# moxime/joint-vae

Hardware: AMD Instinct MI355X
Metric: training_images_per_sec (higher is better)
Workload: dtype f32

## Files before the change

### include/jvae_hip.h

```cpp
#ifndef JVAE_HIP_H
#define JVAE_HIP_H

#include <stddef.h>

#ifdef __cplusplus
extern "C" {
#endif

const char* jvae_version(void);

int jvae_gemm_f32(int M, int N, int K, int batch,
                  const float* A, long sAm, long sAk, long sAb,
                  const float* B, long sBk, long sBn, long sBb,
                  float* C, long sCm, long sCn, long sCb,
                  const float* bias, int bias_mode, int flags, int splitk, void* stream);

int jvae_splitk_fold_f32(const float* part, const float* bias, float* y, int S, long MN, int N, int relu, int accumulate,
                         void* stream);

size_t jvae_conv2d_workspace_bytes(int N, int Cin, int H, int W, int Cout, int KH, int KW, int S, int P, int OP,
                                   int transposed);
int jvae_conv2d_set_split_bf16(int mode);
int jvae_conv2d_set_split_shape16(int on);
int jvae_conv2d_out_shape(int H, int W, int KH, int KW, int S, int P, int OP, int transposed, int* OH, int* OW);
int jvae_conv2d_fwd_f32(const float* x, const float* w, const float* bias, float* y,
                        int N, int Cin, int H, int W, int Cout, int KH, int KW, int S, int P, int OP, int transposed,
                        void* ws, size_t ws_bytes, void* stream);
int jvae_conv2d_stats_splits(int N, int Cin, int H, int W, int Cout, int KH, int KW, int S, int P, int OP, int transposed);
int jvae_conv2d_fwd_stats_f32(const float* x, const float* w, const float* bias, float* y, float* stats, int* nsplit,
                              int N, int Cin, int H, int W, int Cout, int KH, int KW, int S, int P, int OP, int transposed,
                              void* ws, size_t ws_bytes, void* stream);
int jvae_conv2d_dgrad_f32(const float* dy, const float* w, float* dx,
                          int N, int Cin, int H, int W, int Cout, int KH, int KW, int S, int P, int OP, int transposed,
                          void* ws, size_t ws_bytes, void* stream);
int jvae_conv2d_wgrad_f32(const float* x, const float* dy, float* dw, float* dbias, int accumulate,
                          int N, int Cin, int H, int W, int Cout, int KH, int KW, int S, int P, int OP, int transposed,
                          void* ws, size_t ws_bytes, void* stream);

int jvae_pack_cache_configure(void* buf, size_t bytes);
int jvae_pack_cache_begin(void* stream, long long owner, const void* const* weights, int n);
int jvae_pack_cache_end(void);
int jvae_pack_cache_pin(void);
int jvae_pack_cache_reset(void);
int jvae_pack_cache_stats(int* entries, long long* hits, long long* misses, long long* refreshes);

size_t jvae_channel_sum_workspace_bytes(int C);
int jvae_channel_sum_f32(const float* t, float* out, int N, int C, int P, int accumulate, void* ws, size_t ws_bytes,
                         void* stream);

size_t jvae_bn_workspace_bytes(int C);
int jvae_bn_plan(int N, int C, int P, int* nsplit, int* nchunk);
int jvae_image_range(int N, int parts, int j, int* nb, int* ne);
int jvae_bn_fwd_f32(const float* x, const float* gamma, const float* beta,
                    float* running_mean, float* running_var, long long* num_batches_tracked,
                    float* y, float* save_mean, float* save_invstd,
                    int N, int C, int P, float momentum, float eps, int training, int relu,
                    void* ws, size_t ws_bytes, void* stream);
int jvae_bn_fwd_ext_f32(const float* x, const float* gamma, const float* beta,
                        float* running_mean, float* running_var, long long* num_batches_tracked,
                        float* y, float* save_mean, float* save_invstd,
                        int N, int C, int P, float momentum, float eps, int training, int relu,
                        const float* ext_stats, int ext_nsplit, const float* ext_pivot,
                        void* ws, size_t ws_bytes, void* stream);
// ... 181 lines not shown
```

### joint-vae_amd/csrc/conv_api.hip

```cpp
#include "common.h"
#include "jvae_internal.h"
#include "conv_dispatch.h"

namespace {

inline ConvRoute route(const ConvGeom& g, int transposed, ConvDir dir, CallFlags f = {}) {
    return jvae_conv_route(g, transposed, dir, CONV_F32, f);
}

bool affine_ok(const ConvGeom& g, int transposed, ConvDir other, const ConvRoute& r) {
    return r.aff_ok && route(g, transposed, other, {false, false, false, 1}).aff_ok;
}

int fwd_f32(const float* x, const float* w, const float* bias, float* y, float* stats, int* nsplit, const InAff* aff,
            int N, int Cin, int H, int W, int Cout, int KH, int KW, int S, int P, int OP, int transposed,
            void* ws, size_t ws_bytes, void* stream) {
    ConvGeom g; int oh, ow;
    if (nsplit) *nsplit = 0;
    if (!jvae_make_geom(N, Cin, H, W, Cout, KH, KW, S, P, OP, transposed, &g, &oh, &ow)) return JVAE_EINVAL;
    const ConvRoute r = route(g, transposed, CONV_FWD, {bias != nullptr, stats != nullptr, false, jvae_aff_kind(aff)});
    if (aff && !affine_ok(g, transposed, CONV_WGRAD, r)) return JVAE_ENOTSUP;
    if (N == 0) return 0;
    if (jvae_ws_short(r, ws, ws_bytes)) return JVAE_EWORKSPACE;
    return jvae_conv_run_fwd(r, g, x, w, bias, y, (float*)ws, ws_bytes, (hipStream_t)stream, stats, nsplit, aff);
// ... 106 lines not shown

int jvae_conv2d_wgrad_f32(const float* x, const float* dy, float* dw, float* dbias, int accumulate,
                          int N, int Cin, int H, int W, int Cout, int KH, int KW, int S, int P, int OP, int transposed,
                          void* ws, size_t ws_bytes, void* stream) {
    return wgrad_f32(x, dy, dw, dbias, accumulate, nullptr, N, Cin, H, W, Cout, KH, KW, S, P, OP, transposed, ws, ws_bytes, stream);
}

size_t jvae_channel_sum_workspace_bytes(int C) { return jvae_channel_sum_ws_bytes(C); }

int jvae_channel_sum_f32(const float* t, float* out, int N, int C, int P, int accumulate, void* ws, size_t ws_bytes,
                         void* stream) {
    if (!t || !out || N < 0 || C <= 0 || P <= 0) return JVAE_EINVAL;
    return jvae_channel_sum(t, out, N, C, P, accumulate, (float*)ws, ws_bytes, (hipStream_t)stream);
}

}
```

### joint-vae_amd/csrc/conv_dispatch.h

```cpp
#pragma once
#include "common.h"
#include "jvae_internal.h"

size_t jvae_conv_generic_ws(const ConvGeom& g);
int jvae_fold_fwd(const ConvGeom& g, const float* xb, const float* w, const float* bias, float* ys,
                  float* ws, size_t ws_bytes, hipStream_t st);
int jvae_fold_bwd(const ConvGeom& g, const float* ys, const float* w, const float* bias, float* xb,
                  float* ws, size_t ws_bytes, hipStream_t st);
int jvae_fold_wgrad(const ConvGeom& g, const float* xb, const float* ys, float* dw,
                    float* ws, size_t ws_bytes, hipStream_t st);
size_t jvae_channel_sum_ws_bytes(int C);
int jvae_channel_sum(const float* t, float* out, int N, int C, int P, int accumulate, float* ws, size_t ws_bytes,
                     hipStream_t st);

bool jvae_conv5_fwd_ok(int Cin, int H, int W, int Cout, int OH, int OW, int S, int P);
size_t jvae_conv5_pack_floats(int Cin, int Cout);
int jvae_conv5_fwd(const float* in, const float* w, int swap, int flip, const float* bias, float* out,
                   int N, int Cin, int H, int W, int Cout, int OW, int S, int P, float* ws, hipStream_t st,
                   float* stats = nullptr, int* nsplit = nullptr, const InAff* aff = nullptr);
int jvae_conv5_fwd_max_splits(int N, int OW);

int jvae_conv5_pack(const float* w, float* wp, int C, int O, int swap, int flip, hipStream_t st);

bool jvae_conv5_x3_ok(int Cin, int H, int W, int Cout, int OH, int OW, int S, int P);
size_t jvae_conv5_x3_pack_bytes(int Cin, int Cout);
int jvae_conv5_x3_set(int mode);
int jvae_conv5_x3_set_shape16(int on);
bool jvae_conv5_x3_enabled();
// ... 76 lines not shown
```

### joint-vae_amd/csrc/conv_generic.hip

```cpp
#include "common.h"
#include "jvae_internal.h"

namespace {

__global__ __launch_bounds__(256) void unfold_kernel(const float* __restrict__ xb, float* __restrict__ col,
                                                     ConvGeom g, int n0, int nimg, long sn, long sk, long sq,
                                                     int kfast) {
    const int Kd = g.Cb * g.KH * g.KW, Ps = g.Hs * g.Ws;
    const long total = (long)nimg * Kd * Ps;
    for (long i = (long)blockIdx.x * blockDim.x + threadIdx.x; i < total; i += (long)gridDim.x * blockDim.x) {
        int n, k, q;
        if (kfast) { k = (int)(i % Kd); long r = i / Kd; n = (int)(r % nimg); q = (int)(r / nimg); }
        else       { q = (int)(i % Ps); long r = i / Ps; k = (int)(r % Kd);  n = (int)(r / Kd); }
        const int kw = k % g.KW, kh = (k / g.KW) % g.KH, cb = k / (g.KW * g.KH);
        const int hs = q / g.Ws, ws = q % g.Ws;
        const int hb = hs * g.S + kh - g.P, wb = ws * g.S + kw - g.P;
        float v = 0.f;
        if (hb >= 0 && hb < g.Hb && wb >= 0 && wb < g.Wb)
            v = xb[(((long)(n0 + n) * g.Cb + cb) * g.Hb + hb) * g.Wb + wb];
        col[(long)n * sn + (long)k * sk + (long)q * sq] = v;
    }
}

template <bool KFAST>
// ... 56 lines not shown
            if (hs >= g.Hs) continue;
            for (int kw = 0; kw < g.KW; ++kw) {
                const int tw = wb + g.P - kw;
                if (tw < 0 || tw % g.S) continue;
                const int ws = tw / g.S;
                if (ws >= g.Ws) continue;
                const int k = (cb * g.KH + kh) * g.KW + kw;
                acc += col[(long)n * sn + (long)k * sk + (long)(hs * g.Ws + ws) * sq];
            }
        }
        xb[(((long)(n0 + n) * g.Cb + cb) * g.Hb + hb) * g.Wb + wb] = acc;
    }
}

__global__ __launch_bounds__(256) void channel_sum_kernel(const float* __restrict__ t, float* __restrict__ partial,
                                                          int N, int C, int P, int nsplit) {
    __shared__ float red[17];
    const int c = blockIdx.x, sp = blockIdx.y;
    const ImageRange ir = image_range(N, nsplit, sp);
    const int nb = ir.nb, ne = ir.ne;
    float s = 0.f;
    if ((P & 3) == 0) {
        const int P4 = P >> 2;
        const long cnt = (long)(ne - nb) * P4;
        for (long i = threadIdx.x; i < cnt; i += blockDim.x) {
            const long n = nb + i / P4, q = i % P4;
            const f32x4 v = *reinterpret_cast<const f32x4*>(t + (n * C + c) * (long)P + q * 4);
            s += (v[0] + v[1]) + (v[2] + v[3]);
        }
    } else {
        const long cnt = (long)(ne - nb) * P;
        for (long i = threadIdx.x; i < cnt; i += blockDim.x) {
            const long n = nb + i / P, q = i % P;
            s += t[(n * C + c) * (long)P + q];
        }
    }
    s = block_sum(s, red);
    if (threadIdx.x == 0) partial[(long)c * nsplit + sp] = s;
}

__global__ void channel_fold_kernel(const float* __restrict__ partial, float* __restrict__ out, int C, int nsplit,
                                    int accumulate) {
    const int c = blockIdx.x * blockDim.x + threadIdx.x;
    if (c >= C) return;
    float s = 0.f;
    for (int k = 0; k < nsplit; ++k) s += partial[(long)c * nsplit + k];
    out[c] = (accumulate ? out[c] : 0.f) + s;
}

inline int fold_slab_images(const ConvGeom& g) {
    const long per = (long)g.Cb * g.Hb * g.Wb;
    long n = ((1L << 31) - 1) / (per > 0 ? per : 1);
    if (const char* e = getenv("JVAE_FOLD_SLAB")) { const long v = atol(e); if (v > 0 && v < n) n = v; }
// ... 187 lines not shown
    }
    const int chunk = chunk_images(g, ws_bytes);
    if (chunk < 1) return JVAE_EWORKSPACE;
    for (int n0 = 0; n0 < g.N; n0 += chunk) {
        const int ni = (g.N - n0 < chunk) ? g.N - n0 : chunk;
        { const int rc = launch_unfold(xb, ws, g, n0, ni, false, st); if (rc) return rc; }
        int rc = jvae_gemm_launch(g.Cs, Kd, Ps, ni, ys + (long)n0 * g.Cs * Ps, Ps, 1, (long)g.Cs * Ps,
                                  ws, 1, Ps, (long)Kd * Ps, dw, Kd, 1, 0, nullptr, 0, 4, 1, st);
        if (rc) return rc;
    }
    return 0;
}

size_t jvae_channel_sum_ws_bytes(int C) { return sizeof(float) * (size_t)(C > 0 ? C : 1) * 64; }

int jvae_channel_sum(const float* t, float* out, int N, int C, int P, int accumulate, float* ws, size_t ws_bytes,
                     hipStream_t st) {
    if (C <= 0) return 0;
    if (N <= 0) {
        if (!accumulate) {
            hipError_t e = hipMemsetAsync(out, 0, sizeof(float) * (size_t)C, st);
            if (e != hipSuccess) return (int)e;
        }
        return 0;
    }
    if (!ws || ws_bytes < jvae_channel_sum_ws_bytes(C)) return JVAE_EWORKSPACE;
    long work = (long)N * P;
    int ns = (int)(work / 4096);
    const int cap = (1024 + C - 1) / C;
    if (ns > cap) ns = cap;
    if (ns > 64) ns = 64;
    if (ns > N) ns = N;
    if (ns < 1) ns = 1;
    hipLaunchKernelGGL(channel_sum_kernel, dim3(C, ns), dim3(256), 0, st, t, ws, N, C, P, ns);
    JVAE_LAUNCH_CHECK();
    hipLaunchKernelGGL(channel_fold_kernel, dim3(cdiv(C, 64)), dim3(64), 0, st, (const float*)ws, out, C, ns, accumulate);
    JVAE_LAUNCH_CHECK();
    return 0;
}
```

### joint-vae_amd/csrc/gemm.hip

```cpp
#include <stdlib.h>
#include "common.h"
#include "conv_x3.h"
#include "jvae_internal.h"
#include "conv_dispatch.h"

namespace {

constexpr int BK = 32;
constexpr int KQ = BK / 4;

struct GemmP {
    const float* A; long sAm, sAk, sAb;
    const float* B; long sBk, sBn, sBb;
    float* C; long sCm, sCn, sCb;
    const float* bias;
    int bias_mode;
    int bias_div;
    int M, N, K;
    int splitk;
    int kchunk;
    int flags;
    long sCsplit;
    int vecA, vecB;
    int xcd;
};

template <bool VEC>
__device__ __forceinline__ f32x4 load4(const float* p, long stride, int i0, int lim, bool row_ok) {
    f32x4 v = {0.f, 0.f, 0.f, 0.f};
    if (!row_ok) return v;
    if (VEC) {
        if (i0 + 3 < lim) return *reinterpret_cast<const f32x4*>(p);
    }
#pragma unroll
    for (int j = 0; j < 4; ++j)
        if (i0 + j < lim) v[j] = p[j * stride];
    return v;
}

template <int BM, int BN, bool AK, bool BNC>
__global__ __launch_bounds__(256) void gemm_kernel(GemmP p) {
    constexpr int LDA = BM + 4, LDB = BN + 4;
    constexpr int WM = BM / 2, WN = BN / 2;
    constexpr int TM = WM / 32, TN = WN / 32;
    constexpr int GA = BM * BK / 4 / 256;
    constexpr int GB = BN * BK / 4 / 256;
    __shared__ float As[BK * LDA];
    __shared__ float Bs[BK * LDB];

    const int tid = threadIdx.x, lane = tid & 63, wave = tid >> 6;
    const int wm0 = (wave >> 1) * WM, wn0 = (wave & 1) * WN;
    const int m0 = blockIdx.y * BM, n0 = blockIdx.x * BN;
    const int batch = blockIdx.z / p.splitk, split = blockIdx.z % p.splitk;
    const int kbeg = split * p.kchunk;
    const int kend = min(p.K, kbeg + p.kchunk);
    const float* A = p.A + (long)batch * p.sAb;
    const float* B = p.B + (long)batch * p.sBb;
    float* C = p.C + (long)batch * p.sCb + ((p.flags & 8) ? (long)split * p.sCsplit : 0L);

    f32x16 acc[TM][TN];
#pragma unroll
    for (int i = 0; i < TM; ++i)
#pragma unroll
        for (int j = 0; j < TN; ++j)
#pragma unroll
            for (int r = 0; r < 16; ++r) acc[i][j][r] = 0.f;

    f32x4 ra[GA], rb[GB];

    auto gload = [&](int k0) {
#pragma unroll
        for (int g = 0; g < GA; ++g) {
            if (AK) {
// ... 69 lines not shown
#pragma unroll
            for (int i = 0; i < TM; ++i)
#pragma unroll
                for (int j = 0; j < TN; ++j)
                    acc[i][j] = __builtin_amdgcn_mfma_f32_32x32x2f32(a[i], b[j], acc[i][j], 0, 0, 0);
        }
    }

    const bool lead = (split == 0) && !(p.flags & 8);
#pragma unroll
    for (int i = 0; i < TM; ++i)
#pragma unroll
        for (int j = 0; j < TN; ++j) {
            const int n = n0 + wn0 + j * 32 + l31;
            if (n >= p.N) continue;
            float bn = (p.bias_mode == 1 && lead) ? p.bias[n / p.bias_div] : 0.f;
#pragma unroll
            for (int r = 0; r < 16; ++r) {
                const int m = m0 + wm0 + i * 32 + (r & 3) + 8 * (r >> 2) + 4 * half;
                if (m >= p.M) continue;
                float v = acc[i][j][r] + bn;
                if (p.bias_mode == 2 && lead) v += p.bias[m];
                float* dst = C + (long)m * p.sCm + (long)n * p.sCn;
                if (p.flags & 8) {
                    *dst = v;
                } else if (p.flags & 4) {
                    atomicAdd(dst, v);
                } else {
                    if (p.flags & 1) v += *dst;
                    if (p.flags & 2) v = fmaxf(v, 0.f);
                    *dst = v;
                }
            }
        }
}

template <int BM, int BN>
int launch_tile(const GemmP& p, int batch, hipStream_t st) {
    dim3 grid(cdiv(p.N, BN), cdiv(p.M, BM), batch * p.splitk), block(256);
    const bool ak = (p.sAk == 1), bnc = (p.sBn == 1);
    if (ak && bnc)       hipLaunchKernelGGL((gemm_kernel<BM, BN, true, true>), grid, block, 0, st, p);
    else if (ak && !bnc) hipLaunchKernelGGL((gemm_kernel<BM, BN, true, false>), grid, block, 0, st, p);
    else if (!ak && bnc) hipLaunchKernelGGL((gemm_kernel<BM, BN, false, true>), grid, block, 0, st, p);
    else                 hipLaunchKernelGGL((gemm_kernel<BM, BN, false, false>), grid, block, 0, st, p);
    JVAE_LAUNCH_CHECK();
    return 0;
}

inline bool aligned16(const void* p) { return (reinterpret_cast<uintptr_t>(p) & 15) == 0; }

typedef __bf16 gx_bf16x8 __attribute__((ext_vector_type(8)));
typedef __bf16 gx_bf16x4 __attribute__((ext_vector_type(4)));
typedef unsigned int gx_u32x2 __attribute__((ext_vector_type(2)));
typedef unsigned int gx_u32x4 __attribute__((ext_vector_type(4)));
// ... 24 lines not shown
    constexpr int KQX = BKX / 4;
    extern __shared__ __attribute__((aligned(16))) unsigned char gx_lds[];
    unsigned char* As = gx_lds;
    unsigned char* Bs = gx_lds + 3 * IA::BYTES;

    const int tid = threadIdx.x, lane = tid & 63, wave = tid >> 6;
    const int half = lane >> 5, l31 = lane & 31;
    const int cg = (lane >> 4) & 1, q4 = (lane & 15) >> 2, pp = lane & 3;
    const int wm0 = (wave >> 1) * 32, wn0 = (wave & 1) * 32;
    unsigned bx = blockIdx.x, by = blockIdx.y, bz = blockIdx.z;
    if (p.xcd) {
        const unsigned lin = (unsigned)xcd_tile(bx + gridDim.x * (by + gridDim.y * bz), gridDim.x * gridDim.y * gridDim.z);
        bx = lin % gridDim.x; by = (lin / gridDim.x) % gridDim.y; bz = lin / (gridDim.x * gridDim.y);
    }
    const int m0 = by * BM, n0 = bx * BN;
    const int batch = bz / p.splitk, split = bz % p.splitk;
    const int kbeg = split * p.kchunk;
    const int kend = min(p.K, kbeg + p.kchunk);
    const float* A = p.A + (long)batch * p.sAb;
    const float* B = p.B + (long)batch * p.sBb;
    float* C = p.C + (long)batch * p.sCb + ((p.flags & 8) ? (long)split * p.sCsplit : 0L);

    f32x16 acc;
#pragma unroll
    for (int r = 0; r < 16; ++r) acc[r] = 0.f;
    f32x4 ra[DEPTH][G4], rb[DEPTH][G4];

    auto coordA = [&](int g, int k0, int* fast, int* slow) {
        if (AK) { *fast = k0 + (tid % KQX) * 4; *slow = m0 + tid / KQX + g * (256 / KQX); }
        else    { *fast = m0 + (tid % 16) * 4;  *slow = k0 + tid / 16 + g * 16; }
    };
    auto coordB = [&](int g, int k0, int* fast, int* slow) {
        if (BNC) { *fast = n0 + (tid % 16) * 4;  *slow = k0 + tid / 16 + g * 16; }
        else     { *fast = k0 + (tid % KQX) * 4; *slow = n0 + tid / KQX + g * (256 / KQX); }
    };
    auto okA = [&](int fast, int slow) { return AK ? (fast < kend && slow < p.M) : (fast + 3 < p.M && slow < kend); };
// ... 110 lines not shown
        }
    } else {
        if (kbeg < kend) gload(0, kbeg);
        for (int k0 = kbeg; k0 < kend; k0 += BKX) {
            __syncthreads();
            lstore(0, k0);
            __syncthreads();
            if (k0 + BKX < kend) gload(0, k0 + BKX);
            multiply();
        }
    }

    const bool lead = (split == 0) && !(p.flags & 8);
    const int n = n0 + wn0 + l31;
    if (n >= p.N) return;
    const float bn = (p.bias_mode == 1 && lead) ? p.bias[n / p.bias_div] : 0.f;
#pragma unroll
    for (int r = 0; r < 16; ++r) {
        const int m = m0 + wm0 + (r & 3) + 8 * (r >> 2) + 4 * half;
        if (m >= p.M) continue;
        float v = acc[r] + bn;
        if (p.bias_mode == 2 && lead) v += p.bias[m];
        float* dst = C + (long)m * p.sCm + (long)n * p.sCn;
        if (p.flags & 8) {
            *dst = v;
        } else if (p.flags & 4) {
            atomicAdd(dst, v);
        } else {
            if (p.flags & 1) v += *dst;
            if (p.flags & 2) v = fmaxf(v, 0.f);
            *dst = v;
        }
    }
}

template <bool AK, bool BNC, int DEPTH>
int launch_x3_variant(const GemmP& p, int batch, hipStream_t st) {
    constexpr int LDS = 3 * (GxImg<AK>::BYTES + GxImg<!BNC>::BYTES);
    static bool attr_set = false;
    if (!attr_set) {
        hipError_t e = hipFuncSetAttribute(reinterpret_cast<const void*>(&gemm_x3_kernel<AK, BNC, DEPTH>),
                                           hipFuncAttributeMaxDynamicSharedMemorySize, LDS);
        if (e != hipSuccess) return (int)e;
        attr_set = true;
    }
    dim3 grid(cdiv(p.N, 64), cdiv(p.M, 64), batch * p.splitk), block(256);
    hipLaunchKernelGGL((gemm_x3_kernel<AK, BNC, DEPTH>), grid, block, LDS, st, p);
    JVAE_LAUNCH_CHECK();
    return 0;
}

template <bool AK, bool BNC>
int launch_x3_ab(const GemmP& p, int batch, hipStream_t st) {
    const bool deep = p.vecA && p.vecB && p.K % 4 == 0
                      && (AK || p.M % 4 == 0) && (!BNC || p.N % 4 == 0);
    if (deep) return launch_x3_variant<AK, BNC, 3>(p, batch, st);
    return launch_x3_variant<AK, BNC, 1>(p, batch, st);
}

int launch_x3(const GemmP& p0, int batch, hipStream_t st) {
    GemmP p = p0;
// ... 8 lines not shown
inline bool gemm_x3_on(int K) {
    return K >= 64 && jvae_conv5_x3_enabled();
}

}

int jvae_gemm_launch(int M, int N, int K, int batch,
                     const float* A, long sAm, long sAk, long sAb,
                     const float* B, long sBk, long sBn, long sBb,
                     float* C, long sCm, long sCn, long sCb,
                     const float* bias, int bias_mode, int flags, int splitk, hipStream_t st) {
    return jvae_gemm_launch_ex(M, N, K, batch, A, sAm, sAk, sAb, B, sBk, sBn, sBb, C, sCm, sCn, sCb, bias, bias_mode, 1,
                               flags, splitk, st);
}

int jvae_gemm_launch_ex(int M, int N, int K, int batch,
                        const float* A, long sAm, long sAk, long sAb,
                        const float* B, long sBk, long sBn, long sBb,
                        float* C, long sCm, long sCn, long sCb,
                        const float* bias, int bias_mode, int bias_div, int flags, int splitk, hipStream_t st) {
    if (M <= 0 || N <= 0 || batch <= 0) return 0;
    if (K < 0 || !A || !B || !C) return JVAE_EINVAL;
    if (bias_mode && !bias) return JVAE_EINVAL;
    GemmP p;
    p.A = A; p.sAm = sAm; p.sAk = sAk; p.sAb = sAb;
    p.B = B; p.sBk = sBk; p.sBn = sBn; p.sBb = sBb;
    p.C = C; p.sCm = sCm; p.sCn = sCn; p.sCb = sCb;
    p.bias = bias; p.bias_mode = bias_mode; p.bias_div = bias_div > 0 ? bias_div : 1;
    p.M = M; p.N = N; p.K = K;
    if (splitk < 1) splitk = 1;
    int ktiles = cdiv(K, BK);
    if (splitk > ktiles) splitk = ktiles > 0 ? ktiles : 1;
    p.kchunk = cdiv(ktiles, splitk) * BK;
    splitk = K > 0 ? cdiv(K, p.kchunk) : 1;
    p.splitk = splitk;
    p.flags = flags & ~8;
    p.sCsplit = 0;
    if (splitk > 1) {
        if (flags & 2) return JVAE_EINVAL;
        p.flags |= 4;
    }
    const bool ak = (sAk == 1), bnc = (sBn == 1);
    p.vecA = aligned16(A) && (sAb % 4 == 0) && (ak ? (sAm % 4 == 0) : (sAm == 1 && sAk % 4 == 0));
    p.vecB = aligned16(B) && (sBb % 4 == 0) && (bnc ? (sBk % 4 == 0) : (sBk == 1 && sBn % 4 == 0));
    if (gemm_x3_on(K)) return launch_x3(p, batch, st);
    const long tiles128 = (long)cdiv(M, 128) * cdiv(N, 128) * batch * splitk;
    if (M > 64 && N > 64 && tiles128 >= 512) return launch_tile<128, 128>(p, batch, st);
    return launch_tile<64, 64>(p, batch, st);
}

int jvae_gemm_launch_part(int M, int N, int K, int batch,
                          const float* A, long sAm, long sAk, long sAb,
                          const float* B, long sBk, long sBn, long sBb,
                          float* part, long sCm, long sCn, long sCb, long sCsplit, int want_splits, int* splits,
                          hipStream_t st) {
    if (splits) *splits = 0;
    if (M <= 0 || N <= 0 || batch <= 0) return 0;
    if (K <= 0 || !A || !B || !part || !splits) return JVAE_EINVAL;
    GemmP p;
    p.A = A; p.sAm = sAm; p.sAk = sAk; p.sAb = sAb;
    p.B = B; p.sBk = sBk; p.sBn = sBn; p.sBb = sBb;
    p.C = part; p.sCm = sCm; p.sCn = sCn; p.sCb = sCb;
    p.bias = nullptr; p.bias_mode = 0; p.bias_div = 1;
    p.M = M; p.N = N; p.K = K;
    int splitk = want_splits < 1 ? 1 : want_splits;
    const int ktiles = cdiv(K, BK);
    if (splitk > ktiles) splitk = ktiles;
    p.kchunk = cdiv(ktiles, splitk) * BK;
    splitk = cdiv(K, p.kchunk);
    p.splitk = splitk;
    p.flags = 8;
    p.sCsplit = sCsplit;
    const bool ak = (sAk == 1), bnc = (sBn == 1);
    p.vecA = aligned16(A) && (sAb % 4 == 0) && (ak ? (sAm % 4 == 0) : (sAm == 1 && sAk % 4 == 0));
    p.vecB = aligned16(B) && (sBb % 4 == 0) && (bnc ? (sBk % 4 == 0) : (sBk == 1 && sBn % 4 == 0));
    *splits = splitk;
    if (gemm_x3_on(K)) return launch_x3(p, batch, st);
    return launch_tile<64, 64>(p, batch, st);
}

__global__ __launch_bounds__(256) void splitk_fold_kernel(const float* __restrict__ part, const float* __restrict__ bias,
                                                          float* __restrict__ y, int S, long MN, int N, int relu,
                                                          int accumulate, int bias_div) {
    for (long i = (long)blockIdx.x * blockDim.x + threadIdx.x; i < MN; i += (long)gridDim.x * blockDim.x) {
        float v = bias ? bias[(i / bias_div) % N] : 0.f;
        for (int s = 0; s < S; ++s) v += part[(long)s * MN + i];
        if (accumulate) v += y[i];
        y[i] = relu ? fmaxf(v, 0.f) : v;
    }
}

__global__ __launch_bounds__(256) void splitk_fold_qn_kernel(const float* __restrict__ part, const float* __restrict__ bias,
                                                             float* __restrict__ y, int S, int N, int Cs, int Ps) {
    const long total = (long)Ps * N * Cs;
    for (long i = (long)blockIdx.x * blockDim.x + threadIdx.x; i < total; i += (long)gridDim.x * blockDim.x) {
        const int cs = (int)(i % Cs);
        const long r = i / Cs;
        const int n = (int)(r % N), q = (int)(r / N);
// ... 5 lines not shown

int jvae_splitk_fold_qn(const float* part, const float* bias, float* y, int S, int N, int Cs, int Ps, hipStream_t st) {
    const long total = (long)Ps * N * Cs;
    if (total == 0) return 0;
    const int blocks = (int)((total + 255) / 256 > 4096 ? 4096 : (total + 255) / 256);
    hipLaunchKernelGGL(splitk_fold_qn_kernel, dim3(blocks), dim3(256), 0, st, part, bias, y, S, N, Cs, Ps);
    JVAE_LAUNCH_CHECK();
    return 0;
}

int jvae_splitk_fold(const float* part, const float* bias, float* y, int S, long MN, int N, int relu, int accumulate,
                     hipStream_t st, int bias_div) {
    if (MN == 0) return 0;
    const int blocks = (int)((MN + 255) / 256 > 4096 ? 4096 : (MN + 255) / 256);
    hipLaunchKernelGGL(splitk_fold_kernel, dim3(blocks), dim3(256), 0, st, part, bias, y, S, MN, N, relu, accumulate,
                       bias_div > 0 ? bias_div : 1);
    JVAE_LAUNCH_CHECK();
    return 0;
}

extern "C" int jvae_splitk_fold_f32(const float* part, const float* bias, float* y, int S, long MN, int N, int relu,
                                    int accumulate, void* stream) {
    if (!part || !y || S < 1 || MN < 0 || N < 1) return JVAE_EINVAL;
    return jvae_splitk_fold(part, bias, y, S, MN, N, relu, accumulate, (hipStream_t)stream);
}

extern "C" int jvae_gemm_f32(int M, int N, int K, int batch,
                             const float* A, long sAm, long sAk, long sAb,
                             const float* B, long sBk, long sBn, long sBb,
                             float* C, long sCm, long sCn, long sCb,
                             const float* bias, int bias_mode, int flags, int splitk, void* stream) {
    return jvae_gemm_launch(M, N, K, batch, A, sAm, sAk, sAb, B, sBk, sBn, sBb, C, sCm, sCn, sCb,
                            bias, bias_mode, flags, splitk, (hipStream_t)stream);
}
```

### joint-vae_amd/jvae_hip/lib.py

```python
import ctypes
import os
from ctypes import c_char_p, c_float, c_int, c_long, c_longlong, c_size_t, c_void_p, POINTER

import torch

_HERE = os.path.dirname(os.path.abspath(__file__))
LIB_PATH = os.environ.get('JVAE_HIP_LIB') or os.path.join(_HERE, 'libjvae_hip.so')

_lib = None

P = c_void_p
_SIGS = {
    'jvae_version': (c_char_p, []),
    'jvae_gemm_f32': (c_int, [c_int] * 4 + [P, c_long, c_long, c_long] * 3 + [P, c_int, c_int, c_int, P]),
    'jvae_splitk_fold_f32': (c_int, [P, P, P, c_int, c_long, c_int, c_int, c_int, P]),
    'jvae_conv2d_workspace_bytes': (c_size_t, [c_int] * 11),
    'jvae_conv2d_set_split_bf16': (c_int, [c_int]),
    'jvae_conv2d_set_split_shape16': (c_int, [c_int]),
    'jvae_conv2d_out_shape': (c_int, [c_int] * 8 + [POINTER(c_int), POINTER(c_int)]),
    'jvae_conv2d_fwd_f32': (c_int, [P, P, P, P] + [c_int] * 11 + [P, c_size_t, P]),
    'jvae_conv2d_stats_splits': (c_int, [c_int] * 11),
    'jvae_conv2d_fwd_stats_f32': (c_int, [P, P, P, P, P, POINTER(c_int)] + [c_int] * 11 + [P, c_size_t, P]),
    'jvae_conv2d_dgrad_f32': (c_int, [P, P, P] + [c_int] * 11 + [P, c_size_t, P]),
    'jvae_conv2d_wgrad_f32': (c_int, [P, P, P, P, c_int] + [c_int] * 11 + [P, c_size_t, P]),
    'jvae_b8_pack_f32': (c_int, [P, P, c_int, c_int, c_long, P]),
    'jvae_b8_unpack_f32': (c_int, [P, P, c_int, c_int, c_long, c_int, P]),
    'jvae_conv2d_native_b8': (c_int, [c_int] * 11),
    'jvae_conv2d_workspace_bytes_b8': (c_size_t, [c_int] * 11),
    'jvae_conv2d_stats_splits_b8': (c_int, [c_int] * 11),
    'jvae_conv2d_fwd_b8': (c_int, [P, P, P, P, c_int, P, POINTER(c_int)] + [c_int] * 11 + [P, c_size_t, P]),
# ... 13 lines not shown
    'jvae_conv2d_wgrad_aff_b8': (c_int, [P, P, P, P, c_int, P, P, c_int] + [c_int] * 11 + [P, c_size_t, P]),
    'jvae_relu_fwd_b8': (c_int, [P, P, c_long, P]),
    'jvae_relu_bwd_b8': (c_int, [P, P, P, c_long, P]),
    'jvae_bn_finalize_f32': (c_int, [P] * 10 + [c_int, c_int, c_int, c_float, c_float, c_int, P, c_int, P, P, c_size_t, P]),
    'jvae_conv2d_affine_ok': (c_int, [c_int] * 11),
    'jvae_conv2d_fwd_aff_f32': (c_int, [P, P, P, P, P, POINTER(c_int), P, P, c_int] + [c_int] * 11 + [P, c_size_t, P]),
    'jvae_conv2d_wgrad_aff_f32': (c_int, [P, P, P, P, c_int, P, P, c_int] + [c_int] * 11 + [P, c_size_t, P]),
    'jvae_pack_cache_configure': (c_int, [P, c_size_t]),
    'jvae_pack_cache_begin': (c_int, [P, c_longlong, P, c_int]),
    'jvae_pack_cache_end': (c_int, []),
    'jvae_pack_cache_pin': (c_int, []),
    'jvae_pack_cache_reset': (c_int, []),
    'jvae_pack_cache_stats': (c_int, [POINTER(c_int), POINTER(c_longlong), POINTER(c_longlong), POINTER(c_longlong)]),
    'jvae_channel_sum_workspace_bytes': (c_size_t, [c_int]),
    'jvae_channel_sum_f32': (c_int, [P, P, c_int, c_int, c_int, c_int, P, c_size_t, P]),
    'jvae_bn_workspace_bytes': (c_size_t, [c_int]),
    'jvae_bn_plan': (c_int, [c_int, c_int, c_int, POINTER(c_int), POINTER(c_int)]),
    'jvae_image_range': (c_int, [c_int, c_int, c_int, POINTER(c_int), POINTER(c_int)]),
    'jvae_bn_fwd_f32': (c_int, [P] * 9 + [c_int, c_int, c_int, c_float, c_float, c_int, c_int, P, c_size_t, P]),
    'jvae_bn_fwd_ext_f32': (c_int, [P] * 9 + [c_int, c_int, c_int, c_float, c_float, c_int, c_int, P, c_int, P, P, c_size_t, P]),
    'jvae_bn_sums_f32': (c_int, [P, P, P, c_int, c_int, c_int, P, c_size_t, P]),
    'jvae_bn_fwd_sync_f32': (c_int, [P] * 9 + [c_int, c_int, c_int, c_float, c_float, c_int, P, P, c_int, P, c_size_t, P]),
    'jvae_bn_bwd_sums_f32': (c_int, [P] * 7 + [c_int, c_int, c_int, c_int, P, c_size_t, P]),
    'jvae_bn_bwd_sync_f32': (c_int, [P] * 8 + [c_int, P, P, P, c_int, c_int, c_int, c_int, c_int, P]),
    'jvae_bn_bwd_f32': (c_int, [P] * 9 + [c_int, c_int, c_int, c_int, c_int, P, c_size_t, P]),
    'jvae_act_fwd_f32': (c_int, [P, P, c_long, c_int, P]),
    'jvae_act_bwd_f32': (c_int, [P, P, P, c_long, c_int, P]),
    'jvae_dict_stats_f32': (c_int, [P, P, c_int, c_int, P]),
    'jvae_latent_fwd_f32': (c_int, [P] * 13 + [c_int] * 6 + [c_float] * 3 + [c_int, c_int, c_float, P]),
    'jvae_latent_bwd_f32': (c_int, [P] * 17 + [c_int] * 6 + [c_float] * 3 + [c_int, c_int, P, c_size_t, P]),
# ... 153 lines not shown
```

### joint-vae_amd/jvae_hip/ops.py

```python
import contextlib
import math
from ctypes import byref, c_int

import torch

from . import lib as L

RELU, SIGMOID, IDENT, LEAKY = 1, 2, 0, 3
BN_ACT = {IDENT: 0, RELU: 1, LEAKY: 2}
OVERLAP_WGRAD = True
ACT_KIND = {'relu': RELU, 'sigmoid': SIGMOID, 'linear': IDENT, 'leaky': LEAKY, None: IDENT}


def _c(t):
    return t if t.is_contiguous() else t.contiguous()


def _f32(t, what):
    if t.dtype != torch.float32:
        raise L.JvaeHipError(f'{what}: fp32 expected, got {t.dtype}')
    return t


def _grad_slot(param):
# ... 100 lines not shown
            if slot is not None:
                gw = None
        if ctx.has_bias and ctx.needs_input_grad[2]:
            slot = _grad_slot(ctx.b_ref)
            if slot is not None:
                channel_sum(gy, R, O, 1, out=slot, accumulate=True)
            else:
                gb = channel_sum(gy, R, O, 1)
        return gx, gw, gb, None


def linear(x, w, b=None, act=IDENT):
    return _Linear.apply(x, w, b, act)


_GEOM_CACHE = {}


def _geom_query(name, geom):
    key = (name, geom)
    r = _GEOM_CACHE.get(key)
    if r is None:
        _GEOM_CACHE[key] = r = getattr(L.load(), name)(*geom)
    return r


class ConvSpec:
    __slots__ = ('cin', 'cout', 'k', 's', 'p', 'op', 'transposed')

    def __init__(self, cin, cout, k, s, p, op=0, transposed=False):
# ... 839 lines not shown
```

### joint-vae_amd/module/vae_layers/layers.py

```python
import logging
import math

import numpy as np
import torch
from torch import nn
from torch.nn import Parameter

from jvae_hip import ops
from jvae_compat import texify_str
from module.priors import build_prior
from .misc import activation_layers, ACT_OF_MODULE


def _sigma_kind(is_rmse, coded, learned, decay):
    for kind, on in (('rmse', is_rmse), ('coded', coded), ('learned', learned), ('decayed', decay)):
        if on:
            return kind
    return 'fixed'


class Sigma(Parameter):

    @staticmethod
    def __new__(cls, value=None, sdim=1, input_dim=False, learned=False, is_rmse=False, is_log=False, **_):
# ... 245 lines not shown
    def capacity(self):
        m = self.prior.mean
        C = self.num_labels
        d2 = torch.cdist(m, m).pow(2)
        return math.log(C) - torch.exp(-d2 / 4).sum(0).log().sum() / C

    def dict_min_distance(self):
        m = self.prior.mean
        C = self.num_labels
        guard = 2 * m.norm(dim=1).max() * torch.eye(C, device=m.device)
        return (torch.cdist(m, m) + guard).min()

    def heads(self, x, y=None):
        u = x if y is None else torch.cat((x, y), dim=-1)
        u = self.dense_projs(u)
        return u, self.dense_mean(u), (None if self.forced_variance else self.dense_log_var(u))

    def encode(self, x, y_onehot, labels, kl_var_weighting=1., epsilon=None):
        u, mu, lv_raw = self.heads(x, y_onehot)
        K = mu.shape[-1]
        batch = mu.shape[:-1]
        mu2 = mu.reshape(-1, K)
        n = mu2.shape[0]
        pr = self.prior
        if epsilon is None:
            epsilon = draw_epsilon(self._sampling_size, mu.shape, mu.device, self.sampling.distribution)
        lab, means, T = pr._kernel_operands(labels if pr.conditional else None, n, mu.device)
        forced = math.log(self.forced_variance) if self.forced_variance else None
        raw2 = mu2 if lv_raw is None else lv_raw.reshape(-1, K)
        lv, z, kl, dist, vkl, dzd = ops.latent(mu2, raw2, epsilon.reshape(epsilon.shape[0], n, K), lab, means, T,
                                               prior=pr.distribution, var_dim=pr.var_dim, tau=pr._tau,
# ... 28 lines not shown
```

Measured before the change: 139,500.

## Batch mean and log-variance heads into paired GEMM and channel-sum launches

Adds grouped GEMM, split-K fold and channel-sum kernels that handle two independent operands in one launch via an extra grid dimension, and routes the encoder's dense_mean and dense_log_var linear layers through a new paired autograd function. The goal is to halve kernel launches for the small latent-head linears in both forward and backward. Channel-sum also gains a single-slice path that writes output directly and skips the fold kernel. The added per-block group selection is a small extra cost, and the paired path requires both heads to have matching shapes and gradient flags.

```diff
diff --git a/include/jvae_hip.h b/include/jvae_hip.h
--- a/include/jvae_hip.h
+++ b/include/jvae_hip.h
@@ -17,6 +17,14 @@
 
 int jvae_splitk_fold_f32(const float* part, const float* bias, float* y, int S, long MN, int N, int relu, int accumulate,
                          void* stream);
+
+int jvae_gemm_pair_f32(int M, int N, int K, int batch,
+                       const float* A0, const float* A1, long sAm, long sAk, long sAb,
+                       const float* B0, const float* B1, long sBk, long sBn, long sBb,
+                       float* C0, float* C1, long sCm, long sCn, long sCb,
+                       const float* bias0, const float* bias1, int bias_mode, int flags, void* stream);
+int jvae_splitk_fold_pair_f32(const float* part0, const float* part1, const float* bias0, const float* bias1,
+                              float* y0, float* y1, int S, long MN, int N, int relu, int accumulate, void* stream);
 
 size_t jvae_conv2d_workspace_bytes(int N, int Cin, int H, int W, int Cout, int KH, int KW, int S, int P, int OP,
                                    int transposed);
@@ -47,6 +55,8 @@
 size_t jvae_channel_sum_workspace_bytes(int C);
 int jvae_channel_sum_f32(const float* t, float* out, int N, int C, int P, int accumulate, void* ws, size_t ws_bytes,
                          void* stream);
+int jvae_channel_sum_pair_f32(const float* t0, const float* t1, float* out0, float* out1, int N, int C, int P, int accumulate,
+                              void* ws, size_t ws_bytes, void* stream);
 
 size_t jvae_bn_workspace_bytes(int C);
 int jvae_bn_plan(int N, int C, int P, int* nsplit, int* nchunk);
diff --git a/joint-vae_amd/csrc/conv_api.hip b/joint-vae_amd/csrc/conv_api.hip
--- a/joint-vae_amd/csrc/conv_api.hip
+++ b/joint-vae_amd/csrc/conv_api.hip
@@ -144,4 +144,10 @@
     return jvae_channel_sum(t, out, N, C, P, accumulate, (float*)ws, ws_bytes, (hipStream_t)stream);
 }
 
+int jvae_channel_sum_pair_f32(const float* t0, const float* t1, float* out0, float* out1, int N, int C, int P, int accumulate,
+                              void* ws, size_t ws_bytes, void* stream) {
+    if (!t0 || !t1 || !out0 || !out1 || N < 0 || C <= 0 || P <= 0) return JVAE_EINVAL;
+    return jvae_channel_sum_pair(t0, t1, out0, out1, N, C, P, accumulate, (float*)ws, ws_bytes, (hipStream_t)stream);
 }
+
+}
diff --git a/joint-vae_amd/csrc/conv_dispatch.h b/joint-vae_amd/csrc/conv_dispatch.h
--- a/joint-vae_amd/csrc/conv_dispatch.h
+++ b/joint-vae_amd/csrc/conv_dispatch.h
@@ -12,6 +12,8 @@
 size_t jvae_channel_sum_ws_bytes(int C);
 int jvae_channel_sum(const float* t, float* out, int N, int C, int P, int accumulate, float* ws, size_t ws_bytes,
                      hipStream_t st);
+int jvae_channel_sum_pair(const float* t0, const float* t1, float* out0, float* out1, int N, int C, int P, int accumulate,
+                          float* ws, size_t ws_bytes, hipStream_t st);
 
 bool jvae_conv5_fwd_ok(int Cin, int H, int W, int Cout, int OH, int OW, int S, int P);
 size_t jvae_conv5_pack_floats(int Cin, int Cout);
diff --git a/joint-vae_amd/csrc/conv_generic.hip b/joint-vae_amd/csrc/conv_generic.hip
--- a/joint-vae_amd/csrc/conv_generic.hip
+++ b/joint-vae_amd/csrc/conv_generic.hip
@@ -94,9 +94,11 @@
 }
 
 __global__ __launch_bounds__(256) void channel_sum_kernel(const float* __restrict__ t, float* __restrict__ partial,
-                                                          int N, int C, int P, int nsplit) {
+                                                          int N, int C, int P, int nsplit, float* __restrict__ out,
+                                                          int accumulate, const float* __restrict__ t1, float* __restrict__ out1) {
     __shared__ float red[17];
     const int c = blockIdx.x, sp = blockIdx.y;
+    if (blockIdx.z) { t = t1; out = out1; }
     const ImageRange ir = image_range(N, nsplit, sp);
     const int nb = ir.nb, ne = ir.ne;
     float s = 0.f;
@@ -116,7 +118,14 @@
         }
     }
     s = block_sum(s, red);
-    if (threadIdx.x == 0) partial[(long)c * nsplit + sp] = s;
+    if (threadIdx.x != 0) return;
+    if (out) {
+        float f = 0.f;
+        f += s;
+        out[c] = (accumulate ? out[c] : 0.f) + f;
+    } else {
+        partial[(long)c * nsplit + sp] = s;
+    }
 }
 
 __global__ void channel_fold_kernel(const float* __restrict__ partial, float* __restrict__ out, int C, int nsplit,
@@ -334,6 +343,16 @@
 
 size_t jvae_channel_sum_ws_bytes(int C) { return sizeof(float) * (size_t)(C > 0 ? C : 1) * 64; }
 
+inline int channel_sum_slices(int N, int C, int P) {
+    long work = (long)N * P;
+    int ns = (int)(work / 4096);
+    const int cap = (1024 + C - 1) / C;
+    if (ns > cap) ns = cap;
+    if (ns > 64) ns = 64;
+    if (ns > N) ns = N;
+    return ns < 1 ? 1 : ns;
+}
+
 int jvae_channel_sum(const float* t, float* out, int N, int C, int P, int accumulate, float* ws, size_t ws_bytes,
                      hipStream_t st) {
     if (C <= 0) return 0;
@@ -345,16 +364,29 @@
         return 0;
     }
     if (!ws || ws_bytes < jvae_channel_sum_ws_bytes(C)) return JVAE_EWORKSPACE;
-    long work = (long)N * P;
-    int ns = (int)(work / 4096);
-    const int cap = (1024 + C - 1) / C;
-    if (ns > cap) ns = cap;
-    if (ns > 64) ns = 64;
-    if (ns > N) ns = N;
-    if (ns < 1) ns = 1;
-    hipLaunchKernelGGL(channel_sum_kernel, dim3(C, ns), dim3(256), 0, st, t, ws, N, C, P, ns);
+    const int ns = channel_sum_slices(N, C, P);
+    if (ns == 1) {
+        hipLaunchKernelGGL(channel_sum_kernel, dim3(C, 1), dim3(256), 0, st, t, (float*)nullptr, N, C, P, 1, out, accumulate,
+                           (const float*)nullptr, (float*)nullptr);
+        JVAE_LAUNCH_CHECK();
+        return 0;
+    }
+    hipLaunchKernelGGL(channel_sum_kernel, dim3(C, ns), dim3(256), 0, st, t, ws, N, C, P, ns, (float*)nullptr, 0,
+                       (const float*)nullptr, (float*)nullptr);
     JVAE_LAUNCH_CHECK();
     hipLaunchKernelGGL(channel_fold_kernel, dim3(cdiv(C, 64)), dim3(64), 0, st, (const float*)ws, out, C, ns, accumulate);
     JVAE_LAUNCH_CHECK();
     return 0;
 }
+
+int jvae_channel_sum_pair(const float* t0, const float* t1, float* out0, float* out1, int N, int C, int P, int accumulate,
+                          float* ws, size_t ws_bytes, hipStream_t st) {
+    if (C > 0 && N > 0 && channel_sum_slices(N, C, P) == 1) {
+        hipLaunchKernelGGL(channel_sum_kernel, dim3(C, 1, 2), dim3(256), 0, st, t0, (float*)nullptr, N, C, P, 1, out0, accumulate,
+                           t1, out1);
+        JVAE_LAUNCH_CHECK();
+        return 0;
+    }
+    const int rc = jvae_channel_sum(t0, out0, N, C, P, accumulate, ws, ws_bytes, st);
+    return rc ? rc : jvae_channel_sum(t1, out1, N, C, P, accumulate, ws, ws_bytes, st);
+}
diff --git a/joint-vae_amd/csrc/gemm.hip b/joint-vae_amd/csrc/gemm.hip
--- a/joint-vae_amd/csrc/gemm.hip
+++ b/joint-vae_amd/csrc/gemm.hip
@@ -23,6 +23,8 @@
     long sCsplit;
     int vecA, vecB;
     int xcd;
+    int groups;
+    const float* A1; const float* B1; float* C1; const float* bias1;
 };
 
 template <bool VEC>
@@ -51,12 +53,14 @@
     const int tid = threadIdx.x, lane = tid & 63, wave = tid >> 6;
     const int wm0 = (wave >> 1) * WM, wn0 = (wave & 1) * WN;
     const int m0 = blockIdx.y * BM, n0 = blockIdx.x * BN;
-    const int batch = blockIdx.z / p.splitk, split = blockIdx.z % p.splitk;
+    const int zper = gridDim.z / p.groups, group = blockIdx.z / zper, zi = blockIdx.z % zper;
+    const int batch = zi / p.splitk, split = zi % p.splitk;
     const int kbeg = split * p.kchunk;
     const int kend = min(p.K, kbeg + p.kchunk);
-    const float* A = p.A + (long)batch * p.sAb;
-    const float* B = p.B + (long)batch * p.sBb;
-    float* C = p.C + (long)batch * p.sCb + ((p.flags & 8) ? (long)split * p.sCsplit : 0L);
+    const float* A = (group ? p.A1 : p.A) + (long)batch * p.sAb;
+    const float* B = (group ? p.B1 : p.B) + (long)batch * p.sBb;
+    float* C = (group ? p.C1 : p.C) + (long)batch * p.sCb + ((p.flags & 8) ? (long)split * p.sCsplit : 0L);
+    const float* bias = group ? p.bias1 : p.bias;
 
     f32x16 acc[TM][TN];
 #pragma unroll
@@ -156,13 +160,13 @@
         for (int j = 0; j < TN; ++j) {
             const int n = n0 + wn0 + j * 32 + l31;
             if (n >= p.N) continue;
-            float bn = (p.bias_mode == 1 && lead) ? p.bias[n / p.bias_div] : 0.f;
+            float bn = (p.bias_mode == 1 && lead) ? bias[n / p.bias_div] : 0.f;
 #pragma unroll
             for (int r = 0; r < 16; ++r) {
                 const int m = m0 + wm0 + i * 32 + (r & 3) + 8 * (r >> 2) + 4 * half;
                 if (m >= p.M) continue;
                 float v = acc[i][j][r] + bn;
-                if (p.bias_mode == 2 && lead) v += p.bias[m];
+                if (p.bias_mode == 2 && lead) v += bias[m];
                 float* dst = C + (long)m * p.sCm + (long)n * p.sCn;
                 if (p.flags & 8) {
                     *dst = v;
@@ -179,7 +183,7 @@
 
 template <int BM, int BN>
 int launch_tile(const GemmP& p, int batch, hipStream_t st) {
-    dim3 grid(cdiv(p.N, BN), cdiv(p.M, BM), batch * p.splitk), block(256);
+    dim3 grid(cdiv(p.N, BN), cdiv(p.M, BM), p.groups * batch * p.splitk), block(256);
     const bool ak = (p.sAk == 1), bnc = (p.sBn == 1);
     if (ak && bnc)       hipLaunchKernelGGL((gemm_kernel<BM, BN, true, true>), grid, block, 0, st, p);
     else if (ak && !bnc) hipLaunchKernelGGL((gemm_kernel<BM, BN, true, false>), grid, block, 0, st, p);
@@ -234,12 +238,16 @@
         bx = lin % gridDim.x; by = (lin / gridDim.x) % gridDim.y; bz = lin / (gridDim.x * gridDim.y);
     }
     const int m0 = by * BM, n0 = bx * BN;
+    const unsigned zper = gridDim.z / p.groups;
+    const int group = bz / zper;
+    bz %= zper;
     const int batch = bz / p.splitk, split = bz % p.splitk;
     const int kbeg = split * p.kchunk;
     const int kend = min(p.K, kbeg + p.kchunk);
-    const float* A = p.A + (long)batch * p.sAb;
-    const float* B = p.B + (long)batch * p.sBb;
-    float* C = p.C + (long)batch * p.sCb + ((p.flags & 8) ? (long)split * p.sCsplit : 0L);
+    const float* A = (group ? p.A1 : p.A) + (long)batch * p.sAb;
+    const float* B = (group ? p.B1 : p.B) + (long)batch * p.sBb;
+    float* C = (group ? p.C1 : p.C) + (long)batch * p.sCb + ((p.flags & 8) ? (long)split * p.sCsplit : 0L);
+    const float* bias = group ? p.bias1 : p.bias;
 
     f32x16 acc;
 #pragma unroll
@@ -380,13 +388,13 @@
     const bool lead = (split == 0) && !(p.flags & 8);
     const int n = n0 + wn0 + l31;
     if (n >= p.N) return;
-    const float bn = (p.bias_mode == 1 && lead) ? p.bias[n / p.bias_div] : 0.f;
+    const float bn = (p.bias_mode == 1 && lead) ? bias[n / p.bias_div] : 0.f;
 #pragma unroll
     for (int r = 0; r < 16; ++r) {
         const int m = m0 + wm0 + (r & 3) + 8 * (r >> 2) + 4 * half;
         if (m >= p.M) continue;
         float v = acc[r] + bn;
-        if (p.bias_mode == 2 && lead) v += p.bias[m];
+        if (p.bias_mode == 2 && lead) v += bias[m];
         float* dst = C + (long)m * p.sCm + (long)n * p.sCn;
         if (p.flags & 8) {
             *dst = v;
@@ -410,7 +418,7 @@
         if (e != hipSuccess) return (int)e;
         attr_set = true;
     }
-    dim3 grid(cdiv(p.N, 64), cdiv(p.M, 64), batch * p.splitk), block(256);
+    dim3 grid(cdiv(p.N, 64), cdiv(p.M, 64), p.groups * batch * p.splitk), block(256);
     hipLaunchKernelGGL((gemm_x3_kernel<AK, BNC, DEPTH>), grid, block, LDS, st, p);
     JVAE_LAUNCH_CHECK();
     return 0;
@@ -449,15 +457,22 @@
                                flags, splitk, st);
 }
 
-int jvae_gemm_launch_ex(int M, int N, int K, int batch,
-                        const float* A, long sAm, long sAk, long sAb,
-                        const float* B, long sBk, long sBn, long sBb,
-                        float* C, long sCm, long sCn, long sCb,
-                        const float* bias, int bias_mode, int bias_div, int flags, int splitk, hipStream_t st) {
+namespace {
+
+int gemm_launch_groups(int M, int N, int K, int batch,
+                       const float* A, long sAm, long sAk, long sAb,
+                       const float* B, long sBk, long sBn, long sBb,
+                       float* C, long sCm, long sCn, long sCb,
+                       const float* bias, int bias_mode, int bias_div, int flags, int splitk,
+                       const float* A1, const float* B1, float* C1, const float* bias1, hipStream_t st) {
     if (M <= 0 || N <= 0 || batch <= 0) return 0;
     if (K < 0 || !A || !B || !C) return JVAE_EINVAL;
     if (bias_mode && !bias) return JVAE_EINVAL;
+    const bool pair = A1 || B1 || C1;
+    if (pair && (!A1 || !B1 || !C1 || (bias_mode && !bias1))) return JVAE_EINVAL;
     GemmP p;
+    p.groups = pair ? 2 : 1;
+    p.A1 = A1; p.B1 = B1; p.C1 = C1; p.bias1 = bias1;
     p.A = A; p.sAm = sAm; p.sAk = sAk; p.sAb = sAb;
     p.B = B; p.sBk = sBk; p.sBn = sBn; p.sBb = sBb;
     p.C = C; p.sCm = sCm; p.sCn = sCn; p.sCb = sCb;
@@ -478,10 +493,25 @@
     const bool ak = (sAk == 1), bnc = (sBn == 1);
     p.vecA = aligned16(A) && (sAb % 4 == 0) && (ak ? (sAm % 4 == 0) : (sAm == 1 && sAk % 4 == 0));
     p.vecB = aligned16(B) && (sBb % 4 == 0) && (bnc ? (sBk % 4 == 0) : (sBk == 1 && sBn % 4 == 0));
+    if (pair) {
+        p.vecA = p.vecA && aligned16(A1);
+        p.vecB = p.vecB && aligned16(B1);
+    }
     if (gemm_x3_on(K)) return launch_x3(p, batch, st);
     const long tiles128 = (long)cdiv(M, 128) * cdiv(N, 128) * batch * splitk;
     if (M > 64 && N > 64 && tiles128 >= 512) return launch_tile<128, 128>(p, batch, st);
     return launch_tile<64, 64>(p, batch, st);
+}
+
+}
+
+int jvae_gemm_launch_ex(int M, int N, int K, int batch,
+                        const float* A, long sAm, long sAk, long sAb,
+                        const float* B, long sBk, long sBn, long sBb,
+                        float* C, long sCm, long sCn, long sCb,
+                        const float* bias, int bias_mode, int bias_div, int flags, int splitk, hipStream_t st) {
+    return gemm_launch_groups(M, N, K, batch, A, sAm, sAk, sAb, B, sBk, sBn, sBb, C, sCm, sCn, sCb, bias, bias_mode, bias_div,
+                              flags, splitk, nullptr, nullptr, nullptr, nullptr, st);
 }
 
 int jvae_gemm_launch_part(int M, int N, int K, int batch,
@@ -493,6 +523,8 @@
     if (M <= 0 || N <= 0 || batch <= 0) return 0;
     if (K <= 0 || !A || !B || !part || !splits) return JVAE_EINVAL;
     GemmP p;
+    p.groups = 1;
+    p.A1 = nullptr; p.B1 = nullptr; p.C1 = nullptr; p.bias1 = nullptr;
     p.A = A; p.sAm = sAm; p.sAk = sAk; p.sAb = sAb;
     p.B = B; p.sBk = sBk; p.sBn = sBn; p.sBb = sBb;
     p.C = part; p.sCm = sCm; p.sCn = sCn; p.sCb = sCb;
@@ -516,7 +548,9 @@
 
 __global__ __launch_bounds__(256) void splitk_fold_kernel(const float* __restrict__ part, const float* __restrict__ bias,
                                                           float* __restrict__ y, int S, long MN, int N, int relu,
-                                                          int accumulate, int bias_div) {
+                                                          int accumulate, int bias_div, const float* __restrict__ part1,
+                                                          const float* __restrict__ bias1, float* __restrict__ y1) {
+    if (blockIdx.y) { part = part1; bias = bias1; y = y1; }
     for (long i = (long)blockIdx.x * blockDim.x + threadIdx.x; i < MN; i += (long)gridDim.x * blockDim.x) {
         float v = bias ? bias[(i / bias_div) % N] : 0.f;
         for (int s = 0; s < S; ++s) v += part[(long)s * MN + i];
@@ -552,7 +586,18 @@
     if (MN == 0) return 0;
     const int blocks = (int)((MN + 255) / 256 > 4096 ? 4096 : (MN + 255) / 256);
     hipLaunchKernelGGL(splitk_fold_kernel, dim3(blocks), dim3(256), 0, st, part, bias, y, S, MN, N, relu, accumulate,
-                       bias_div > 0 ? bias_div : 1);
+                       bias_div > 0 ? bias_div : 1, (const float*)nullptr, (const float*)nullptr, (float*)nullptr);
+    JVAE_LAUNCH_CHECK();
+    return 0;
+}
+
+extern "C" int jvae_splitk_fold_pair_f32(const float* part0, const float* part1, const float* bias0, const float* bias1,
+                                         float* y0, float* y1, int S, long MN, int N, int relu, int accumulate, void* stream) {
+    if (!part0 || !part1 || !y0 || !y1 || S < 1 || MN < 0 || N < 1 || (!bias0) != (!bias1)) return JVAE_EINVAL;
+    if (MN == 0) return 0;
+    const int blocks = (int)((MN + 255) / 256 > 4096 ? 4096 : (MN + 255) / 256);
+    hipLaunchKernelGGL(splitk_fold_kernel, dim3(blocks, 2), dim3(256), 0, (hipStream_t)stream, part0, bias0, y0, S, MN, N, relu,
+                       accumulate, 1, part1, bias1, y1);
     JVAE_LAUNCH_CHECK();
     return 0;
 }
@@ -571,3 +616,13 @@
     return jvae_gemm_launch(M, N, K, batch, A, sAm, sAk, sAb, B, sBk, sBn, sBb, C, sCm, sCn, sCb,
                             bias, bias_mode, flags, splitk, (hipStream_t)stream);
 }
+
+extern "C" int jvae_gemm_pair_f32(int M, int N, int K, int batch,
+                                  const float* A0, const float* A1, long sAm, long sAk, long sAb,
+                                  const float* B0, const float* B1, long sBk, long sBn, long sBb,
+                                  float* C0, float* C1, long sCm, long sCn, long sCb,
+                                  const float* bias0, const float* bias1, int bias_mode, int flags, void* stream) {
+    if (!A1 || !B1 || !C1) return JVAE_EINVAL;
+    return gemm_launch_groups(M, N, K, batch, A0, sAm, sAk, sAb, B0, sBk, sBn, sBb, C0, sCm, sCn, sCb, bias0, bias_mode, 1,
+                              flags, 1, A1, B1, C1, bias1, (hipStream_t)stream);
+}
diff --git a/joint-vae_amd/jvae_hip/lib.py b/joint-vae_amd/jvae_hip/lib.py
--- a/joint-vae_amd/jvae_hip/lib.py
+++ b/joint-vae_amd/jvae_hip/lib.py
@@ -14,6 +14,8 @@
     'jvae_version': (c_char_p, []),
     'jvae_gemm_f32': (c_int, [c_int] * 4 + [P, c_long, c_long, c_long] * 3 + [P, c_int, c_int, c_int, P]),
     'jvae_splitk_fold_f32': (c_int, [P, P, P, c_int, c_long, c_int, c_int, c_int, P]),
+    'jvae_gemm_pair_f32': (c_int, [c_int] * 4 + [P, P, c_long, c_long, c_long] * 3 + [P, P, c_int, c_int, P]),
+    'jvae_splitk_fold_pair_f32': (c_int, [P] * 6 + [c_int, c_long, c_int, c_int, c_int, P]),
     'jvae_conv2d_workspace_bytes': (c_size_t, [c_int] * 11),
     'jvae_conv2d_set_split_bf16': (c_int, [c_int]),
     'jvae_conv2d_set_split_shape16': (c_int, [c_int]),
@@ -57,6 +59,7 @@
     'jvae_pack_cache_stats': (c_int, [POINTER(c_int), POINTER(c_longlong), POINTER(c_longlong), POINTER(c_longlong)]),
     'jvae_channel_sum_workspace_bytes': (c_size_t, [c_int]),
     'jvae_channel_sum_f32': (c_int, [P, P, c_int, c_int, c_int, c_int, P, c_size_t, P]),
+    'jvae_channel_sum_pair_f32': (c_int, [P] * 4 + [c_int, c_int, c_int, c_int, P, c_size_t, P]),
     'jvae_bn_workspace_bytes': (c_size_t, [c_int]),
     'jvae_bn_plan': (c_int, [c_int, c_int, c_int, POINTER(c_int), POINTER(c_int)]),
     'jvae_image_range': (c_int, [c_int, c_int, c_int, POINTER(c_int), POINTER(c_int)]),
diff --git a/joint-vae_amd/jvae_hip/ops.py b/joint-vae_amd/jvae_hip/ops.py
--- a/joint-vae_amd/jvae_hip/ops.py
+++ b/joint-vae_amd/jvae_hip/ops.py
@@ -138,6 +138,97 @@
     return _Linear.apply(x, w, b, act)
 
 
+def _gemm_pair(M, N, K, A, sA, B, sB, C, sC, bias=(None, None), bias_mode=0, flags=0, batch=1):
+    rc = L.load().jvae_gemm_pair_f32(M, N, K, batch, L.ptr(A[0]), L.ptr(A[1]), *sA, L.ptr(B[0]), L.ptr(B[1]), *sB,
+                                     L.ptr(C[0]), L.ptr(C[1]), *sC, L.ptr(bias[0]), L.ptr(bias[1]), bias_mode, flags,
+                                     L.stream_ptr())
+    L.check(rc, 'jvae_gemm_pair_f32')
+
+
+class _LinearPair(torch.autograd.Function):
+
+    @staticmethod
+    def forward(ctx, x, w0, b0, w1, b1):
+        x2 = _c(_f32(x, 'linear').reshape(-1, x.shape[-1]))
+        ws = (_c(w0), _c(w1))
+        bs = (b0, b1)
+        R, I = x2.shape
+        O = w0.shape[0]
+        y = torch.empty((2, R, O), device=x.device, dtype=torch.float32)
+        S = _linear_split(R, O, I)
+        if S > 1:
+            part = torch.empty((2, S, R, O), device=x.device, dtype=torch.float32)
+            Ks = I // S
+            _gemm_pair(R, O, Ks, (x2, x2), (I, 1, Ks), ws, (1, I, Ks), part, (O, 1, R * O), batch=S)
+            L.check(L.load().jvae_splitk_fold_pair_f32(L.ptr(part[0]), L.ptr(part[1]), L.ptr(b0), L.ptr(b1), L.ptr(y[0]),
+                                                       L.ptr(y[1]), S, R * O, O, 0, 0, L.stream_ptr()),
+                    'jvae_splitk_fold_pair_f32')
+        else:
+            _gemm_pair(R, O, I, (x2, x2), (I, 1, 0), ws, (1, I, 0), y, (O, 1, 0), bias=bs, bias_mode=1 if b0 is not None else 0)
+        ctx.save_for_backward(x2, *ws)
+        ctx.has_bias = b0 is not None
+        ctx.xshape = x.shape
+        ctx.w_refs, ctx.b_refs = (w0, w1), bs
+        return y[0].reshape(*x.shape[:-1], O), y[1].reshape(*x.shape[:-1], O)
+
+    @staticmethod
+    def backward(ctx, gy0, gy1):
+        x2, w0, w1 = ctx.saved_tensors
+        lib = L.load()
+        R, I = x2.shape
+        O = w0.shape[0]
+        gys = (_c(gy0.reshape(R, O)), _c(gy1.reshape(R, O)))
+        dev = x2.device
+        gx = None
+        gws = [None, None]
+        gbs = [None, None]
+        if ctx.needs_input_grad[0]:
+            gx = torch.empty((R, I), device=dev, dtype=torch.float32)
+            gemm(R, I, O, gys[0], (O, 1, 0), w0, (I, 1, 0), gx, (I, 1, 0))
+            gemm(R, I, O, gys[1], (O, 1, 0), w1, (I, 1, 0), gx, (I, 1, 0), flags=1)
+            gx = gx.reshape(ctx.xshape)
+        need_w = (ctx.needs_input_grad[1], ctx.needs_input_grad[3])
+        if all(need_w):
+            slots = [_grad_slot(w) for w in ctx.w_refs]
+            gw = [s if s is not None else torch.zeros((O, I), device=dev, dtype=torch.float32) for s in slots]
+            S = _linear_split(O, I, R)
+            if S > 1:
+                part = torch.empty((2, S, O, I), device=dev, dtype=torch.float32)
+                Rs = R // S
+                _gemm_pair(O, I, Rs, gys, (1, O, Rs * O), (x2, x2), (I, 1, Rs * I), part, (I, 1, O * I), batch=S)
+                L.check(lib.jvae_splitk_fold_pair_f32(L.ptr(part[0]), L.ptr(part[1]), None, None, L.ptr(gw[0]), L.ptr(gw[1]),
+                                                      S, O * I, I, 0, 1, L.stream_ptr()), 'jvae_splitk_fold_pair_f32')
+            else:
+                _gemm_pair(O, I, R, gys, (1, O, 0), (x2, x2), (I, 1, 0), gw, (I, 1, 0), flags=1)
+            gws = [None if s is not None else g for s, g in zip(slots, gw)]
+        elif any(need_w):
+            raise L.JvaeHipError('linear pair: both weights or neither must require a gradient')
+        need_b = (ctx.needs_input_grad[2], ctx.needs_input_grad[4])
+        if ctx.has_bias and all(need_b):
+            slots = [_grad_slot(b) for b in ctx.b_refs]
+            direct = all(s is not None for s in slots)
+            gb = slots if direct else [torch.empty(O, device=dev, dtype=torch.float32) for _ in slots]
+            wsb = L.workspace(lib.jvae_channel_sum_workspace_bytes(O), dev)
+            L.check(lib.jvae_channel_sum_pair_f32(L.ptr(gys[0]), L.ptr(gys[1]), L.ptr(gb[0]), L.ptr(gb[1]), R, O, 1,
+                                                  int(direct), L.ptr(wsb), wsb.numel(), L.stream_ptr()), 'channel_sum_pair')
+            if not direct:
+                gbs = gb
+        elif ctx.has_bias and any(need_b):
+            raise L.JvaeHipError('linear pair: both biases or neither must require a gradient')
+        return gx, gws[0], gbs[0], gws[1], gbs[1]
+
+
+def linear_pair_ok(x, lin0, lin1):
+    w0, w1, b0, b1 = lin0.weight, lin1.weight, lin0.bias, lin1.bias
+    return (x.is_cuda and w0.shape == w1.shape and (b0 is None) == (b1 is None)
+            and w0.dtype == w1.dtype == torch.float32 and w0.requires_grad == w1.requires_grad
+            and (b0 is None or b0.requires_grad == b1.requires_grad))
+
+
+def linear_pair(x, w0, b0, w1, b1):
+    return _LinearPair.apply(x, w0, b0, w1, b1)
+
+
 _GEOM_CACHE = {}
 
 
diff --git a/joint-vae_amd/module/vae_layers/layers.py b/joint-vae_amd/module/vae_layers/layers.py
--- a/joint-vae_amd/module/vae_layers/layers.py
+++ b/joint-vae_amd/module/vae_layers/layers.py
@@ -283,7 +283,13 @@
     def heads(self, x, y=None):
         u = x if y is None else torch.cat((x, y), dim=-1)
         u = self.dense_projs(u)
-        return u, self.dense_mean(u), (None if self.forced_variance else self.dense_log_var(u))
+        if self.forced_variance:
+            return u, self.dense_mean(u), None
+        if ops.linear_pair_ok(u, self.dense_mean, self.dense_log_var):
+            mu, lv = ops.linear_pair(u, self.dense_mean.weight, self.dense_mean.bias,
+                                     self.dense_log_var.weight, self.dense_log_var.bias)
+            return u, mu, lv
+        return u, self.dense_mean(u), self.dense_log_var(u)
 
     def encode(self, x, y_onehot, labels, kl_var_weighting=1., epsilon=None):
         u, mu, lv_raw = self.heads(x, y_onehot)
```

Measured after the change: 140,700, median of 6. No clear change (+0.9%).
